# YukunXia/SuperPoint-Stereo-Visual-Odometry

Measured on AMD Instinct MI355X. Metric: stereo frames/sec (1241x376 KITTI), higher is better.
Workload: dtype f32

## Files before the change

### superpoint-stereo-visual-odometry_amd/csrc/conv_wino4.hip.h

```cpp
#pragma once
#include <hip/hip_runtime.h>
#include <stdint.h>
#include <type_traits>
#include <utility>
#include <vector>
#include "conv_mfma.hip.h"

#ifndef WINO4_LEAD
#define WINO4_LEAD 6
#endif
#ifndef WINO4_PRIO
#define WINO4_PRIO 1
#endif
#ifndef WINO4_H1_STEPS
#define WINO4_H1_STEPS 6
#endif
#ifndef WINO4_H1_START
#define WINO4_H1_START 3
#endif
#ifndef WINO4_H1_STRIDE
#define WINO4_H1_STRIDE 5
#endif
#ifndef WINO4_H2_START
#define WINO4_H2_START 4
#endif
#ifndef WINO4_H2_STRIDE
#define WINO4_H2_STRIDE 8
#endif
#ifndef WINO4_ITEM_LEAD
#define WINO4_ITEM_LEAD 6
#endif
#ifndef WINO4_ABL
#define WINO4_ABL 0
#endif

#ifndef SPVO_STATIC_BANDS
#define SPVO_STATIC_BANDS 1
#endif

namespace spvo {

template <int TB>
struct Wino4TileT {
  static constexpr int CK = 4, TH = 8 * TB, TW = 32, LW = TW + 8, LH = TH + 2, NT = 16 * TB, NTH = 256 * TB;
  static constexpr int IN_FLOATS = CK * LH * LW;
  static constexpr int U_FLOATS = 36 * CK * CO_TILE;
  static constexpr int V_FLOATS = 10 * TB * 64 * 4;
  static constexpr int RAW_OFF = 0, U_OFF = 2 * IN_FLOATS, V_OFF = U_OFF + 2 * U_FLOATS;
  static constexpr int LDS_BYTES = (V_OFF + 2 * V_FLOATS) * 4 + 16;
};
using Wino4Tile = Wino4TileT<2>;

inline std::vector<float> pack_conv_weights_wino4(const float *w, const float *bias, int cout, int cin) {
  constexpr int CK = Wino4Tile::CK;
  const int co_tiles = (cout + CO_TILE - 1) / CO_TILE, nch = cin / CK;
  std::vector<float> out((size_t)co_tiles * nch * Wino4Tile::U_FLOATS + (size_t)co_tiles * CO_TILE, 0.f);
  static const double G[6][3] = {{0.25, 0, 0}, {-1.0 / 6, -1.0 / 6, -1.0 / 6}, {-1.0 / 6, 1.0 / 6, -1.0 / 6},
                                 {1.0 / 24, 1.0 / 12, 1.0 / 6}, {1.0 / 24, -1.0 / 12, 1.0 / 6}, {0, 0, 1}};
  for (int ct = 0; ct < co_tiles; ++ct)
    for (int o = 0; o < CO_TILE; ++o) {
      const int co = ct * CO_TILE + o;
      if (co >= cout) continue;
      out[(size_t)co_tiles * nch * Wino4Tile::U_FLOATS + co] = bias[co];
// ... 1 lines not shown
        const float *g = w + ((size_t)co * cin + ci) * 9;
        double t[6][3];
        for (int a = 0; a < 6; ++a)
          for (int k = 0; k < 3; ++k) t[a][k] = G[a][0] * g[0 * 3 + k] + G[a][1] * g[1 * 3 + k] + G[a][2] * g[2 * 3 + k];
        float *slab = out.data() + ((size_t)ct * nch + ci / CK) * Wino4Tile::U_FLOATS;
        const int lane = 16 * (ci % CK) + (o & 15), cq = o >> 4;
        for (int a = 0; a < 6; ++a)
          for (int b = 0; b < 6; ++b) {
            const int pos = 18 * (b / 3) + 3 * a + b % 3;
            slab[(((pos >> 2) * 4 + cq) * 64 + lane) * 4 + (pos & 3)] = (float)(t[a][0] * G[b][0] + t[a][1] * G[b][1] + t[a][2] * G[b][2]);
          }
      }
    }
  return out;
}

__device__ __forceinline__ void wino4_in6(const float x0, const float x1, const float x2, const float x3, const float x4, const float x5, float (&o)[6]) {
  const float e = fmaf(-4.f, x2, x4), od = fmaf(-4.f, x1, x3), e2 = x4 - x2, o2 = x3 - x1;
  o[0] = fmaf(4.f, x0, fmaf(-5.f, x2, x4));
  o[1] = e + od;
  o[2] = e - od;
  o[3] = fmaf(2.f, o2, e2);
  o[4] = fmaf(-2.f, o2, e2);
  o[5] = fmaf(4.f, x1, fmaf(-5.f, x3, x5));
}
__device__ __forceinline__ void wino4_out4(const float m0, const float m1, const float m2, const float m3, const float m4, const float m5, float (&y)[4]) {
  const float a = m1 + m2, b = m1 - m2, c = m3 + m4, d = m3 - m4;
  y[0] = (m0 + a) + c;
  y[1] = fmaf(2.f, d, b);
  y[2] = fmaf(4.f, c, a);
  y[3] = fmaf(8.f, d, b) + m5;
}

typedef float wino4_f32x2 __attribute__((ext_vector_type(2)));
__device__ __forceinline__ void wino4_out4(const wino4_f32x2 m0, const wino4_f32x2 m1, const wino4_f32x2 m2, const wino4_f32x2 m3, const wino4_f32x2 m4,
                                           const wino4_f32x2 m5, wino4_f32x2 (&y)[4]) {
  const wino4_f32x2 a = m1 + m2, b = m1 - m2, c = m3 + m4, d = m3 - m4;
  y[0] = (m0 + a) + c;
  y[1] = __builtin_elementwise_fma(wino4_f32x2{2.f, 2.f}, d, b);
  y[2] = __builtin_elementwise_fma(wino4_f32x2{4.f, 4.f}, c, a);
  y[3] = __builtin_elementwise_fma(wino4_f32x2{8.f, 8.f}, d, b) + m5;
}

constexpr int wino4_b_piece(int p) { return 5 * (p / 18) + ((p % 18) >> 2); }
constexpr bool wino4_slot_reads_a(int q) { return (q & 3) == 0; }
constexpr bool wino4_slot_reads_b(int q) { return q == 0 || wino4_b_piece(q) != wino4_b_piece(q - 1); }
constexpr int wino4_reads_before(int q_end) {
  int n = 0;
  for (int q = 0; q < q_end && q < 36; ++q) n += (wino4_slot_reads_a(q) ? 1 : 0) + (wino4_slot_reads_b(q) ? 1 : 0);
  return n;
}
constexpr int wino4_first_slot_b(int piece) { return 18 * (piece / 5) + 4 * (piece % 5); }
constexpr int wino4_wait_count(int p, int lead) {
  const int issued = wino4_reads_before(p + lead);
  const int qa = p & ~3, qb = wino4_first_slot_b(wino4_b_piece(p));
  const int ia = wino4_reads_before(qa);
  const int ib = wino4_reads_before(qb) + (wino4_slot_reads_a(qb) ? 1 : 0);
  const int n = issued - 1 - (ia > ib ? ia : ib);
  return n < 0 ? 0 : (n > 15 ? 15 : n);
}
template <class F, int... P>
__device__ __forceinline__ void wino4_for_each(F &&f, std::integer_sequence<int, P...>) { (f(std::integral_constant<int, P>{}), ...); }

template <bool POOL, bool RELU, int TAG = 0, int TB = 2, int ITEM = 2>
__global__ __launch_bounds__(256 * TB, TB) void conv_wino4_kernel(const ConvArgs a) {
  using T = Wino4TileT<TB>;
  constexpr int CK = T::CK, LW = T::LW, LH = T::LH, LW4 = LW / 4, NTH = T::NTH;
  constexpr int IN_V4 = T::IN_FLOATS / 4;
  constexpr int U_V4 = T::U_FLOATS / 4;
  constexpr bool NEW_ITEM = ITEM != 0 && !(WINO4_ABL & 8);
  constexpr int NIT_U = (U_V4 + NTH - 1) / NTH;
  typedef float f32x2 __attribute__((ext_vector_type(2)));
  typedef float f32x4v __attribute__((ext_vector_type(4)));

  extern __shared__ __attribute__((aligned(16))) float smem[];

  const int tid = threadIdx.x;
  const int lane = tid & 63;
  const int c16 = lane & 15, g4 = lane >> 4;
  const int wave = __builtin_amdgcn_readfirstlane(tid >> 6);
  const int cq = wave & 3, tb = wave >> 2;
  const size_t in_plane = (size_t)a.in_hp * a.in_wp;
  const size_t out_plane = (size_t)a.out_hp * a.out_wp;
  const int n_tiles = a.tiles_x * a.tiles_y * a.co_tiles * a.batch;

  struct TileRef { const float *in_base, *w_base; int x0, y0, ct, img; };
  auto decode = [&](int id) {
    TileRef t;
    const int tx = id % a.tiles_x;
    id /= a.tiles_x;
    const int ty = id % a.tiles_y;
    id /= a.tiles_y;
    t.ct = id % a.co_tiles;
    t.img = id / a.co_tiles;
    t.x0 = tx * T::TW;
    t.y0 = ty * T::TH;
    t.in_base = a.in + ((size_t)t.img * a.in_ctot + a.in_coff) * in_plane + (size_t)(t.y0 + PADY - 1) * a.in_wp + (t.x0 + PADX - 4);
    t.w_base = a.wpack + (size_t)t.ct * a.n_chunks * T::U_FLOATS;
    return t;
  };

  auto raw_piece_off = [&](int idx) {
    idx = min(idx, IN_V4 - 1);
    const int ci = idx / (LH * LW4);
    const int rem = idx - ci * (LH * LW4);
    const int r = rem / LW4;
    const int q = rem - r * LW4;
    return 4u * (unsigned)(ci * (int)in_plane + r * a.in_wp + q * 4);
  };
  constexpr int R0 = NTH - 256;
  unsigned roff0 = raw_piece_off(tid), roff1 = raw_piece_off(NTH + (tid - R0));
  const bool raw2 = tid >= R0 && NTH + (tid - R0) < IN_V4;
  auto issue_raw = [&](const TileRef &t, int chunk, float *buf) {
    const char *inb = reinterpret_cast<const char *>(t.in_base + (size_t)chunk * CK * in_plane);
    glds16(reinterpret_cast<const float *>(inb + roff0), buf + (wave * 64) * 4);
    if (raw2) glds16(reinterpret_cast<const float *>(inb + roff1), buf + (NTH + (wave - R0 / 64) * 64) * 4);
  };
  unsigned uoff = 16u * (unsigned)tid;
  auto issue_u = [&](const TileRef &t, int chunk, float *buf) {
    const char *wb = reinterpret_cast<const char *>(t.w_base + (size_t)chunk * T::U_FLOATS);
#pragma unroll
    for (int it = 0; it < NIT_U; ++it)
      if (it < NIT_U - 1 || tid < U_V4 - (NIT_U - 1) * NTH) glds16(reinterpret_cast<const float *>(wb + (uoff + 16u * NTH * it)), buf + (it * NTH + wave * 64) * 4);
  };
  auto issue_raw2 = [&](const TileRef &t, int chunk, float *buf) {
    const char *inb = reinterpret_cast<const char *>(t.in_base + (size_t)chunk * CK * in_plane);
    glds16_sv(inb, roff0, buf + (wave * 64) * 4);
    if (raw2) glds16_sv(inb, roff1, buf + (NTH + (wave - R0 / 64) * 64) * 4);
  };
  auto issue_u2 = [&](const TileRef &t, int chunk, float *buf) {
    const char *wb = reinterpret_cast<const char *>(t.w_base + (size_t)chunk * T::U_FLOATS);
#pragma unroll
    for (int it = 0; it < NIT_U; ++it)
      if (it < NIT_U - 1 || tid < U_V4 - (NIT_U - 1) * NTH) glds16_sv(wb + (size_t)16 * NTH * it, uoff, buf + (it * NTH + wave * 64) * 4);
  };

  const int x_ci = TB == 2 ? (wave & 3) : 2 * (wave & 1) + ((lane >> 4) & 1), x_tile = TB == 2 ? (lane & 31) : (lane & 15), x_h = lane >> 5;
  const int x_trow = x_tile >> 3, x_tcol = x_tile & 7;
  const int raw_off = x_ci * (LH * LW) + (4 * x_trow + 3 * x_h) * LW + 4 * x_tcol + 3;
  const int v_off = x_h * (1280 * TB) + (x_tile >> 4) * 256 + (16 * x_ci + (x_tile & 15)) * 4;
  float xr[3][6];
  f32x4v xa[3];
  float xs0[3], xs1[3];
  f32x2 xs2[3];
  auto xf_step = [&](const float *raw, float *vb, int st) {
    if (st < 3) {
      const float *d = raw + raw_off + st * LW;
      xs0[st] = d[0];
      xa[st] = *reinterpret_cast<const f32x4v *>(d + 1);
      xs1[st] = d[5];
    } else if (st < 6) {
      const int r = st - 3;
      wino4_in6(xs0[r], xa[r][0], xa[r][1], xa[r][2], xa[r][3], xs1[r], xr[r]);
    } else if (st == 6) {
#pragma unroll
      for (int r = 0; r < 3; ++r)
#pragma unroll
        for (int c = 0; c < 3; ++c) {
          typedef unsigned u32x2s __attribute__((ext_vector_type(2)));
          const u32x2s sw = __builtin_amdgcn_permlane32_swap(__float_as_uint(xr[r][c]), __float_as_uint(xr[r][c + 3]), false, false);
          xr[r][c] = __uint_as_float(sw[0]);
          xr[r][c + 3] = __uint_as_float(sw[1]);
        }
    } else {
      const int c = st - 7;
      float o[6];
      wino4_in6(xr[0][c], xr[1][c], xr[2][c], xr[0][c + 3], xr[1][c + 3], xr[2][c + 3], o);
// ... 21 lines not shown
  };
  auto all_done = [&]() {
    if (a.sched && tid == 0 && atomicAdd(a.sched + 8, 1) == (int)gridDim.x - 1)
      for (int k = 0; k < 9; ++k) a.sched[k] = 0;
  };
  int *const sched_slot = reinterpret_cast<int *>(smem + (T::LDS_BYTES - 16) / 4);
  int tile_id = SPVO_STATIC_BANDS ? wgs_before(band) + ((int)blockIdx.x >> 3) : (int)blockIdx.x;
  if (a.sched) {
    tile_id = band_lo(band) + (blockIdx.x >> 3);
    if (tile_id >= band_hi(band)) {
      if (tid == 0) *sched_slot = steal();
      __syncthreads();
      tile_id = *sched_slot;
      __syncthreads();
    }
  }
  if (tile_id >= n_tiles) {
    all_done();
    return;
  }
  TileRef cur = decode(tile_id);

  int nxt_id = tile_id + gridDim.x;
  int dyn_fetch = 0;
  struct Cursor { TileRef t; int chunk, id; };
  auto advance = [&](Cursor &q) {
    if (++q.chunk == a.n_chunks) {
      asm volatile("" ::: "memory");
      q.chunk = 0;
      q.id = a.sched ? nxt_id : q.id + (int)gridDim.x;
      if (q.id < n_tiles) q.t = decode(q.id);
    }
  };
  Cursor cu{cur, 0, tile_id};
  issue_raw(cu.t, 0, smem + T::RAW_OFF);
  issue_u(cu.t, 0, smem + T::U_OFF);
  advance(cu);
  if (cu.id < n_tiles) issue_raw(cu.t, cu.chunk, smem + T::RAW_OFF + T::IN_FLOATS);
  Cursor cr = cu;
  advance(cr);
  asm volatile("s_waitcnt vmcnt(0)\n\ts_barrier" ::: "memory");
  if (wave < 2 * TB) {
#pragma unroll
    for (int st = 0; st < 10; ++st) xf_step(smem + T::RAW_OFF, smem + T::V_OFF, st);
  } else {
#pragma unroll
    for (int st = 0; st < WINO4_H1_STEPS; ++st) xf_step(smem + T::RAW_OFF + T::IN_FLOATS, smem + T::V_OFF + T::V_FLOATS, st);
  }
  asm volatile("s_waitcnt lgkmcnt(0)\n\ts_barrier" ::: "memory");
  if (cr.id < n_tiles) issue_raw(cr.t, cr.chunk, smem + T::RAW_OFF);
  advance(cr);

#ifdef WINO_STAMPS
  unsigned long long st_dma = 0, st_bar = 0, st_mfma = 0, st_epi = 0, st_items = 0, st_post = 0, st_bar_xf = 0, st_mfma_xf = 0;
  const unsigned long long st_t0 = __builtin_amdgcn_s_memtime(), st_r0 = __builtin_amdgcn_s_memrealtime();
  int st_c = 0;
#endif
  int k = 0;
  bool drained = false;
  constexpr unsigned OOB = 0xFFFFFFFFu;

  while (tile_id < n_tiles) {
    if (a.sched) {
      if (tid == 0) dyn_fetch = band_lo(band) + band_wgs(band) + atomicAdd(a.sched + band, 1);
    } else {
      nxt_id = tile_id + gridDim.x;
    }

    f32x4v acc[36];
    auto item = [&](auto first_tag, bool publish) {
      constexpr bool FIRST = decltype(first_tag)::value;
      const bool XF = NEW_ITEM ? (((wave >> TB) ^ k) & 1) == 0 : __builtin_amdgcn_readfirstlane((wave >> TB) == (k & 1) ? 1 : 0) != 0;
#ifdef WINO_STAMPS
      const unsigned long long ts0 = __builtin_amdgcn_s_memtime();
#endif
      if (!drained) asm volatile("s_waitcnt vmcnt(0)" ::: "memory");
      drained = false;
#ifdef WINO_STAMPS
      const unsigned long long ts1 = __builtin_amdgcn_s_memtime();
#endif
      if (publish && tid == 0) *sched_slot = dyn_fetch < band_hi(band) ? dyn_fetch : n_tiles;
      asm volatile("s_waitcnt lgkmcnt(0)\n\ts_barrier" ::: "memory");
      if (publish) nxt_id = __builtin_amdgcn_readfirstlane(*sched_slot);
#ifdef WINO_STAMPS
      const unsigned long long ts2 = __builtin_amdgcn_s_memtime();
      st_dma += ts1 - ts0; st_bar += ts2 - ts1;
      if (st_c == 1) st_post += ts1 - ts0;
      if (XF) st_bar_xf += ts2 - ts1;
#endif
      const float *ub = smem + T::U_OFF + (k & 1) * T::U_FLOATS;
      const float *vb = smem + T::V_OFF + (k & 1) * T::V_FLOATS;
      float *u_next = smem + T::U_OFF + ((k + 1) & 1) * T::U_FLOATS;
      const float *raw_next2 = smem + T::RAW_OFF + (k & 1) * T::IN_FLOATS;
      float *raw_next3 = smem + T::RAW_OFF + ((k + 1) & 1) * T::IN_FLOATS;
      float *v_next = smem + T::V_OFF + ((k + 1) & 1) * T::V_FLOATS;
      const f32x4v *ub4 = reinterpret_cast<const f32x4v *>(ub) + a_lane;
      const f32x4v *vb4 = reinterpret_cast<const f32x4v *>(vb) + b_lane;
      if constexpr (NEW_ITEM) {
        constexpr int LEAD = WINO4_ITEM_LEAD;
        static_assert(LEAD >= 1 && LEAD <= 36, "WINO4_ITEM_LEAD");
        static_assert(WINO4_PRIO <= 1, "the other priority schedules exist in the ITEM = 0 form only");
        f32x4v av[9], bv[10];
        f32x2 bh[2];
        static_assert(WINO4_H1_STEPS >= 6, "the row reads and the row pass that waits for them run in one item");
        const int xf_s = ((wave >> TB) ^ k ^ 1) & 1;
        auto is_xf = [xf_s]() __attribute__((always_inline)) { int t = xf_s; asm volatile("" : "+s"(t)); return t != 0; };
        const unsigned ra = (unsigned)(uintptr_t)(const __attribute__((address_space(3))) void *)(raw_next2 + raw_off);
        const unsigned ua = (unsigned)(uintptr_t)(const __attribute__((address_space(3))) void *)ub4;
        const unsigned va = (unsigned)(uintptr_t)(const __attribute__((address_space(3))) void *)vb4;
        auto read_slot = [&av, &bv, &bh, ua, va](auto qc) __attribute__((always_inline)) {
          constexpr int q = decltype(qc)::value;
          if constexpr (q < 36 && wino4_slot_reads_a(q)) asm volatile("ds_read_b128 %0, %1 offset:%2" : "=v"(av[q >> 2]) : "v"(ua), "n"((q >> 2) * 256 * 16));
          constexpr int j = wino4_b_piece(q < 36 ? q : 35);
          if constexpr (q < 36 && wino4_slot_reads_b(q) && j % 5 == 4) asm volatile("ds_read_b64 %0, %1 offset:%2" : "=v"(bh[j / 5]) : "v"(va), "n"(j * 64 * TB * 16));
          if constexpr (q < 36 && wino4_slot_reads_b(q) && j % 5 != 4) asm volatile("ds_read_b128 %0, %1 offset:%2" : "=v"(bv[j]) : "v"(va), "n"(j * 64 * TB * 16));
        };
        auto step = [&](auto pc) __attribute__((always_inline)) {
          constexpr int p = decltype(pc)::value;
          constexpr int ph = p / 18, pq = p % 18, pos = 6 * (pq / 3) + 3 * ph + pq % 3, bj = wino4_b_piece(p);
          constexpr bool half = bj % 5 == 4;
          if constexpr (wino4_slot_reads_a(p) || wino4_slot_reads_b(p)) {
            if constexpr (half) asm volatile("s_waitcnt lgkmcnt(%2)" : "+v"(av[p >> 2]), "+v"(bh[bj / 5]) : "n"(wino4_wait_count(p, LEAD)));
            else asm volatile("s_waitcnt lgkmcnt(%2)" : "+v"(av[p >> 2]), "+v"(bv[bj]) : "n"(wino4_wait_count(p, LEAD)));
          }
          const float a_op = av[p >> 2][p & 3];
          float b_op;
          if constexpr (half) b_op = bh[bj / 5][pq & 3];
          else b_op = bv[bj][pq & 3];
#if WINO4_PRIO
          if constexpr (p == 0) asm volatile("s_setprio 3");
          if constexpr (p == 9) asm volatile("s_setprio 2");
          if constexpr (p == 18) asm volatile("s_setprio 1");
          if constexpr (p == 27) asm volatile("s_setprio 0");
#endif
          if (FIRST) acc[pos] = __builtin_amdgcn_mfma_f32_16x16x4f32(a_op, b_op, f32x4v{0.f, 0.f, 0.f, 0.f}, 0, 0, 0);
          else acc[pos] = __builtin_amdgcn_mfma_f32_16x16x4f32(a_op, b_op, acc[pos], 0, 0, 0);
          __builtin_amdgcn_sched_barrier(0);
          if (!(WINO4_ABL & 2) && p == 1 && cu.id < n_tiles) { if constexpr (ITEM == 2) issue_u2(cu.t, cu.chunk, u_next); else issue_u(cu.t, cu.chunk, u_next); }
          if (!(WINO4_ABL & 4) && p == 4 && cr.id < n_tiles) { if constexpr (ITEM == 2) issue_raw2(cr.t, cr.chunk, raw_next3); else issue_raw(cr.t, cr.chunk, raw_next3); }
          read_slot(std::integral_constant<int, p + LEAD>{});
          if constexpr (!(WINO4_ABL & 1) && p >= WINO4_H1_START && p < WINO4_H1_START + WINO4_H1_STEPS * WINO4_H1_STRIDE && (p - WINO4_H1_START) % WINO4_H1_STRIDE == 0) {
            constexpr int st = (p - WINO4_H1_START) / WINO4_H1_STRIDE;
            if (is_xf()) {
              if constexpr (st < 3) {
                asm volatile("ds_read2_b32 %0, %1 offset0:%2 offset1:%3" : "=v"(xs2[st]) : "v"(ra), "n"(st * LW), "n"(st * LW + 5));
                asm volatile("ds_read_b128 %0, %1 offset:%2" : "=v"(xa[st]) : "v"(ra), "n"((st * LW + 1) * 4));
              } else {
                if constexpr (st < 6) {
                  constexpr int p_rd = p - 3 * WINO4_H1_STRIDE;
                  constexpr int n = wino4_reads_before(p + LEAD + 1) - wino4_reads_before(p_rd + LEAD + 1) + 2 * (5 - st);
                  asm volatile("s_waitcnt lgkmcnt(%2)" : "+v"(xs2[st - 3]), "+v"(xa[st - 3]) : "n"(n > 15 ? 15 : n));
                  xs0[st - 3] = xs2[st - 3][0];
                  xs1[st - 3] = xs2[st - 3][1];
                }
                xf_step(raw_next2, v_next, st);
              }
            }
          }
          if constexpr (!(WINO4_ABL & 1) && p >= WINO4_H2_START && p < WINO4_H2_START + (10 - WINO4_H1_STEPS) * WINO4_H2_STRIDE && (p - WINO4_H2_START) % WINO4_H2_STRIDE == 0)
            if (!is_xf()) xf_step(raw_next2, v_next, WINO4_H1_STEPS + (p - WINO4_H2_START) / WINO4_H2_STRIDE);
          __builtin_amdgcn_sched_barrier(0);
        };
        wino4_for_each(read_slot, std::make_integer_sequence<int, LEAD>{});
        wino4_for_each(step, std::make_integer_sequence<int, 36>{});
      } else {
        constexpr int LEAD = WINO4_LEAD;
        f32x4v av[9], bv[10];
        auto b_piece = [](int p) { return 5 * (p / 18) + ((p % 18) >> 2); };
#pragma unroll
        for (int p = 0; p < ((WINO4_ABL & 8) ? 36 : LEAD); ++p) {
          if ((WINO4_ABL & 8) && k > 0) break;
          if ((p & 3) == 0) av[p >> 2] = ub4[(p >> 2) * 256];
          if (p == 0 || b_piece(p) != b_piece(p - 1)) bv[b_piece(p)] = vb4[b_piece(p) * (64 * TB)];
        }
#pragma unroll
        for (int p = 0; p < 36; ++p) {
          const int ph = p / 18, pq = p % 18, pos = 6 * (pq / 3) + 3 * ph + pq % 3;
          const float a_op = av[p >> 2][p & 3], b_op = bv[b_piece(p)][pq & 3];
#if WINO4_PRIO
#if WINO4_PRIO == 1
          if (p == 0) asm volatile("s_setprio 3");
          if (p == 9) asm volatile("s_setprio 2");
          if (p == 18) asm volatile("s_setprio 1");
          if (p == 27) asm volatile("s_setprio 0");
#elif WINO4_PRIO == 2
          if (p == 0) asm volatile("s_setprio 3");
          if (tb == 0) { if (p == 6) asm volatile("s_setprio 2"); if (p == 15) asm volatile("s_setprio 1"); if (p == 24) asm volatile("s_setprio 0"); }
          else { if (p == 12) asm volatile("s_setprio 2"); if (p == 24) asm volatile("s_setprio 1"); }
#elif WINO4_PRIO == 3
          if (p == 0) asm volatile("s_setprio 1");
          if (p == 18) asm volatile("s_setprio 0");
#elif WINO4_PRIO == 4
          if (tb == 0) { if (p == 0) asm volatile("s_setprio 2"); if (p == 12) asm volatile("s_setprio 1"); if (p == 24) asm volatile("s_setprio 0"); }
          else { if (p == 0) asm volatile("s_setprio 3"); if (p == 12) asm volatile("s_setprio 2"); if (p == 24) asm volatile("s_setprio 1"); }
#endif
#endif
          if (FIRST) acc[pos] = __builtin_amdgcn_mfma_f32_16x16x4f32(a_op, b_op, f32x4v{0.f, 0.f, 0.f, 0.f}, 0, 0, 0);
          else acc[pos] = __builtin_amdgcn_mfma_f32_16x16x4f32(a_op, b_op, acc[pos], 0, 0, 0);
          __builtin_amdgcn_sched_barrier(0);
          if (!(WINO4_ABL & 2) && p == 1 && cu.id < n_tiles) issue_u(cu.t, cu.chunk, u_next);
          if (!(WINO4_ABL & 4) && p == 4 && cr.id < n_tiles) issue_raw(cr.t, cr.chunk, raw_next3);
          const int q = p + LEAD;
          if (!(WINO4_ABL & 8) && q < 36) {
            if ((q & 3) == 0) av[q >> 2] = ub4[(q >> 2) * 256];
            if (b_piece(q) != b_piece(q - 1)) bv[b_piece(q)] = vb4[b_piece(q) * (64 * TB)];
          }
          if (!(WINO4_ABL & 1) && XF && p >= WINO4_H1_START && p < WINO4_H1_START + WINO4_H1_STEPS * WINO4_H1_STRIDE && (p - WINO4_H1_START) % WINO4_H1_STRIDE == 0)
            xf_step(raw_next2, v_next, (p - WINO4_H1_START) / WINO4_H1_STRIDE);
          if (!(WINO4_ABL & 1) && !XF && p >= WINO4_H2_START && p < WINO4_H2_START + (10 - WINO4_H1_STEPS) * WINO4_H2_STRIDE && (p - WINO4_H2_START) % WINO4_H2_STRIDE == 0)
            xf_step(raw_next2, v_next, WINO4_H1_STEPS + (p - WINO4_H2_START) / WINO4_H2_STRIDE);
          __builtin_amdgcn_sched_barrier(0);
        }
      }
      advance(cu);
      advance(cr);
      ++k;
#ifdef WINO_STAMPS
      { const unsigned long long dt = __builtin_amdgcn_s_memtime() - ts2; st_mfma += dt; if (XF) st_mfma_xf += dt; }
      ++st_items; ++st_c;
#endif
    };
#ifdef WINO_STAMPS
    st_c = 0;
#endif
    item(std::true_type{}, false);
    for (int c = 1; c < a.n_chunks; ++c) item(std::false_type{}, a.sched != nullptr && c == 1);

#ifdef WINO_STAMPS
    const unsigned long long te0 = __builtin_amdgcn_s_memtime();
#endif
    asm volatile("s_waitcnt vmcnt(0)" ::: "memory");
    drained = true;

    const int co0 = cur.ct * CO_TILE + cq * 16 + 4 * g4;
    float *co_base = a.out + (((size_t)cur.img * a.out_ctot + a.out_coff) + (size_t)cur.ct * CO_TILE + cq * 16) * out_plane;
    const __amdgpu_buffer_rsrc_t rsrc = __builtin_amdgcn_make_buffer_rsrc(co_base, 0, 0x7FFFFFFF, 0x00020000);
    const int oplane = (int)out_plane;
    const int kmax = a.cout - co0;
    const float *bias_p = a.wpack + (size_t)a.co_tiles * a.n_chunks * T::U_FLOATS + min(co0, a.cout - 1);
    const int trow = 2 * tb + (c16 >> 3), tcol = c16 & 7;
    auto relu = [](float v) { return RELU ? __builtin_amdgcn_fmed3f(v, 0.f, __builtin_inff()) : v; };
    const int oy = cur.y0 + 4 * trow, ox = cur.x0 + 4 * tcol;
#pragma unroll
    for (int rp = 0; rp < 2; ++rp) {
      typedef wino4_f32x2 f32x2;
      const f32x2 bias_v = {bias_p[2 * rp < kmax ? 2 * rp : 0], bias_p[2 * rp + 1 < kmax ? 2 * rp + 1 : 0]};
      auto pr = [&](int p) { return f32x2{acc[p][2 * rp], acc[p][2 * rp + 1]}; };
      f32x2 z[6][4];
// ... 67 lines not shown
```

### superpoint-stereo-visual-odometry_amd/csrc/spvo_internal.hip.h

```cpp
#pragma once
#include <hip/hip_runtime.h>

#include <algorithm>
#include <cmath>
#include <cstdarg>
#include <cstdio>
#include <cstdlib>
#include <cstring>
#include <string>
#include <vector>
#include <deque>
#include <functional>
#include <time.h>

#include "../../include/spvo.h"
#include "spvo_types.hip.h"
#include "engine_file.h"

#pragma GCC visibility push(hidden)
#include "dev_buf.h"
namespace spvo { struct BriskLongPair; struct BriskShortPair; }
using namespace spvo;

#include "launch_segments.hip.h"
// ... 13 lines not shown
};
template <class T> using DevBuf = Buf<T, DevMem>;
template <class T> using PinBuf = Buf<T, PinnedMem>;

constexpr int RING = 8;
constexpr int MAX_INFLIGHT = 6;
constexpr int N_SLOTS = 16;
constexpr int N_BIN_SLOTS = 10;
constexpr int N_SIFT_SLOTS = 10;
constexpr int SIFT_SLOT_MAX = 32768;
constexpr int BIN_COUNTER_INTS = 16;
constexpr int HAM_KEY_SHIFT = 22;

struct Tensor {
  int ch = 0, level = 0, H = 0, W = 0, hp = 0, wp = 0;
  bool nhwc = false;
  bool f16 = false;
  bool i8 = false;
  bool s3 = false;
  float scale = 0.f;
  float *d = nullptr;
  float *dr[RING] = {};
  size_t per_image = 0;
};

struct Op {
  int type = 0, in = 0, out = 0, out_c_off = 0, in_c_off = 0, cin = 0, cout = 0, ks = 0, flags = 0;
  int ck = 0, n_chunks = 0, co_tiles = 0, wr = 0, wc = 0;
  int residual = 0;
  bool merged = false;
  bool wino = false;
  bool wino_narrow = false;
  bool wino4 = false;
  int wino4_item = 2;
  bool dominant = false;
  float *d_w = nullptr, *d_b = nullptr, *d_bn_scale = nullptr, *d_bn_shift = nullptr;
  int *d_sched = nullptr;
  _Float16 *d_w16 = nullptr;
  int8_t *d_w8 = nullptr;
  unsigned short *d_ws3 = nullptr;
  int *d_wq32 = nullptr;
  int *d_wsel = nullptr;
  int fused_dw = -1;
  bool fused_stem = false;
  bool fused_away = false;
  float *d_qm = nullptr;
  float inv_s_out = 0.f, s_res = 0.f;
  double flops_per_image = 0;
  int stage = -1;
  mutable int launch_tiles = 0, launch_wgs = 0;
  mutable int launch_block = 0;
};

struct Stage {
  std::string name;
  double total_ms = 0;
  long long calls = 0;
  double flops = 0, bytes = 0;
  double flops_sum = 0, bytes_sum = 0;
};

struct Pending { int stage; hipEvent_t e0, e1; double flops = 0, bytes = 0; };

struct SlotState {
  int n = 0;
  bool filled = false;
  DevBuf<int> d_n;
// ... 642 lines not shown
```

### superpoint-stereo-visual-odometry_amd/csrc/spvo_net_f32.hip

```cpp
#include "spvo_internal.hip.h"
#include "conv_mfma.hip.h"
#include "conv_wino2.hip.h"
#include "conv_wino4.hip.h"
#include "heads.hip.h"

namespace spvo_int {

int prepare_conv_f32(spvo_ctx *c, unsigned i, const float *w, const float *b) {
  Op &op = c->ops[i];
  const Tensor &ti = c->tensors[op.in];
  const bool bn = op.flags & FLAG_BN, add = op.flags & FLAG_ADD, pool = op.flags & FLAG_POOL;
  if (op.cin == 1) {
    if (pool || add) return fail(c, SPVO_ERR_IO, "op %u: single-channel-input layers have no pooling / residual form", i);
    return upload_stem(c, op, w, b);
  }
  op.ck = choose_variant(c, op, ti);
  {
    const bool wino_on = tuning("winograd", 1) != 0;
    const long wtiles = (long)((ti.W + WinoTile::TW - 1) / WinoTile::TW) * ((ti.H + WinoTile::TH - 1) / WinoTile::TH) * op.co_tiles * c->cfg.max_batch;
    const long min_tiles = tuning("winograd_min_tiles", 3 * c->num_cus / 4);
    const bool eligible = wino_on && op.ks == 3 && !bn && !add && (op.cin % WinoTile::CK) == 0 && (!pool || ((ti.H % 2) == 0 && (ti.W % 2) == 0));
    op.wino = eligible && wtiles >= min_tiles;
    if (eligible && !op.wino && tuning("wino_narrow", 1) && (op.cout % 32) == 0 && 3 * wtiles >= min_tiles) op.wino = op.wino_narrow = true;
  }
  const bool dynamic_tiles = tuning("wino_dynamic", 1) != 0;
  int rc;
  if (op.wino && !op.wino_narrow && (op.cin % Wino4Tile::CK) == 0 && (((ti.H | ti.W) & 1) == 0 || !pool) && tuning("wino4", 1)) {
    const long t4 = (long)((ti.W + Wino4Tile::TW - 1) / Wino4Tile::TW) * ((ti.H + Wino4Tile::TH - 1) / Wino4Tile::TH) * op.co_tiles * c->cfg.max_batch;
    if (t4 >= tuning("wino4_min_tiles", 3 * c->num_cus / 4)) {
      op.wino4 = true;
      op.wino4_item = (int)tuning("wino4_item", 2);
      op.ck = Wino4Tile::CK;
      op.n_chunks = op.cin / Wino4Tile::CK;
      if ((rc = upload(c, &op.d_w, pack_conv_weights_wino4(w, b, op.cout, op.cin)))) return rc;
      return dynamic_tiles ? dev_alloc(c, &op.d_sched, 16) : SPVO_OK;
    }
  }
  if (op.wino) {
    op.ck = WinoTile::CK;
    op.n_chunks = op.cin / op.ck;
    if (op.wino_narrow) op.co_tiles = op.cout / 32;
    if ((rc = upload(c, &op.d_w, pack_conv_weights_wino2(w, b, op.cout, op.cin, op.wino_narrow ? 32 : CO_TILE)))) return rc;
    return dynamic_tiles ? dev_alloc(c, &op.d_sched, 16) : SPVO_OK;
  }
  if (op.cin % op.ck) return fail(c, SPVO_ERR_IO, "op %u: cin %d is not a multiple of %d", i, op.cin, op.ck);
  op.n_chunks = op.cin / op.ck;
  std::vector<float> bp((size_t)op.co_tiles * CO_TILE, 0.f);
  for (int o = 0; o < op.cout; ++o) bp[o] = b[o];
  if ((rc = upload(c, &op.d_w, pack_conv_weights(w, b, op.cout, op.cin, op.ks, op.ck)))) return rc;
  return upload(c, &op.d_b, bp);
}

int fuse_tail_f32(spvo_ctx *c, const float *payload, const EngineOp &rp, const EngineOp &rd) {
  const Op &pb = c->ops[c->head_start], &db = c->ops[c->head_start + 1];
  const bool plain = tail_is_plain(c, HEADS_CIN) && !c->tensors[pb.in].nhwc && !c->tensors[db.in].nhwc && !pb.merged && !db.merged &&
                     c->tensors[pb.in].f16 == c->fp16 && c->tensors[db.in].f16 == c->fp16 && (!c->fp16 || ((pb.in_c_off | db.in_c_off) % 8) == 0);
  if (!plain) return SPVO_OK;
  const int rc = upload(c, &c->d_heads_w, pack_heads_weights(payload + rp.w_off, payload + rp.b_off, pb.cout, payload + rd.w_off, payload + rd.b_off, c->fp16));
  if (!rc) c->heads_fused = true;
  return rc;
}

template <int KS, int CK, int WR, int WC, bool POOL, bool RELU, int EPI = 0, int MINW = 1, int TAG = 0>
int launch_conv_instance(spvo_ctx *c, const ConvArgs &args, hipStream_t stream) {
// ... 49 lines not shown

template <bool POOL, bool RELU, int TAG, int ITEM>
int launch_conv_wino4_instance(spvo_ctx *c, const ConvArgs &args, hipStream_t stream) {
  static bool ready[64] = {};
  const int dev = c->cfg.device & 63;
  auto k = conv_wino4_kernel<POOL, RELU, TAG, 2, ITEM>;
  if (!ready[dev]) {
    HIP_TRY(c, hipFuncSetAttribute((const void *)k, hipFuncAttributeMaxDynamicSharedMemorySize, Wino4Tile::LDS_BYTES));
    ready[dev] = true;
  }
  const int n_tiles = args.tiles_x * args.tiles_y * args.co_tiles * args.batch;
  const int rounds = (n_tiles + c->num_cus - 1) / c->num_cus;
  const int grid = (n_tiles + rounds - 1) / rounds;
  ConvArgs a2 = args;
  if (rounds < 2 || args.n_chunks < 5) a2.sched = nullptr;
  hipLaunchKernelGGL(k, dim3(grid), dim3(512), Wino4Tile::LDS_BYTES, stream, a2);
  HIP_TRY(c, hipGetLastError());
  return SPVO_OK;
}

template <int ITEM>
int launch_conv_wino4_sel(spvo_ctx *c, const ConvArgs &args, bool relu, bool pool, bool dominant, hipStream_t stream) {
  if (dominant && relu) return pool ? launch_conv_wino4_instance<true, true, 1, ITEM>(c, args, stream) : launch_conv_wino4_instance<false, true, 1, ITEM>(c, args, stream);
  if (pool) return relu ? launch_conv_wino4_instance<true, true, 0, ITEM>(c, args, stream) : launch_conv_wino4_instance<true, false, 0, ITEM>(c, args, stream);
  return relu ? launch_conv_wino4_instance<false, true, 0, ITEM>(c, args, stream) : launch_conv_wino4_instance<false, false, 0, ITEM>(c, args, stream);
}

int launch_conv_wino4(spvo_ctx *c, const ConvArgs &a, int batch, bool relu, bool pool, bool dominant, int item, hipStream_t stream) {
  ConvArgs args = a;
  args.tiles_x = (a.W + Wino4Tile::TW - 1) / Wino4Tile::TW;
  args.tiles_y = (a.H + Wino4Tile::TH - 1) / Wino4Tile::TH;
  args.batch = batch;
  if (pool && ((a.H | a.W) & 1)) return fail(c, SPVO_ERR_INVALID, "F(4x4) kernel: pooled layer with odd size");
  if (item >= 2) return launch_conv_wino4_sel<2>(c, args, relu, pool, dominant, stream);
  return item == 1 ? launch_conv_wino4_sel<1>(c, args, relu, pool, dominant, stream) : launch_conv_wino4_sel<0>(c, args, relu, pool, dominant, stream);
}

int launch_conv_wino(spvo_ctx *c, const ConvArgs &a, int batch, bool relu, bool pool, bool dominant, bool narrow, hipStream_t stream) {
  ConvArgs args = a;
  args.tiles_x = (a.W + WinoTile::TW - 1) / WinoTile::TW;
  args.tiles_y = (a.H + WinoTile::TH - 1) / WinoTile::TH;
  args.batch = batch;
  return launch_conv_wino_sel(c, args, relu, pool, dominant, narrow, stream);
}

int launch_conv(spvo_ctx *c, const Op &op, int img0, int batch, hipStream_t stream) {
  const Tensor &ti = c->tensors[op.in];
  const Tensor &to = c->tensors[op.out];
  const float *tin = ring_ptr(c, ti, img0);
  float *tout = ring_ptr(c, to, img0);
  const bool relu = op.flags & FLAG_RELU, pool = op.flags & FLAG_POOL;
  const int epi = (op.flags & FLAG_BN) ? 1 : (op.flags & FLAG_ADD) ? 2 : 0;
  if (op.type == OP_DWCONV) {
    dim3 grid((ti.W + 255) / 256, (ti.H + 3) / 4, batch * op.cout);
    if (relu)
      hipLaunchKernelGGL(dwconv3x3_kernel<true>, grid, dim3(256), 0, stream, tin, tout, op.d_w, op.d_b, op.cout, ti.H, ti.W, ti.hp, ti.wp);
    else
      hipLaunchKernelGGL(dwconv3x3_kernel<false>, grid, dim3(256), 0, stream, tin, tout, op.d_w, op.d_b, op.cout, ti.H, ti.W, ti.hp, ti.wp);
    HIP_TRY(c, hipGetLastError());
    return SPVO_OK;
  }
  if (op.cin == 1) {
    dim3 grid((ti.W + 63) / 64, (ti.H + 3) / 4, batch);
#define SPVO_FIRST(KS, RELU) hipLaunchKernelGGL((conv_first_kernel<KS, RELU>), grid, dim3(256), 0, stream, tin, tout, op.d_w, op.d_b, \
                                                op.d_bn_scale, op.d_bn_shift, ti.H, ti.W, ti.hp, ti.wp, to.ch, op.out_c_off, op.cout, 0)
    if (op.ks == 3 && !op.d_bn_scale) {
      dim3 g4((ti.W + 255) / 256, (ti.H + 3) / 4, batch);
// ... 149 lines not shown
```

Before: 1592.

## Add item-3 Winograd F(4x4) path with persistent pointers and LDS address rotation

Adds a new kernel variant (ITEM=3, now the default) that keeps running global pointers for the filter and input DMA instead of recomputing them from tile descriptors, toggles the transform role and LDS buffer addresses by arithmetic swaps, and moves the priority setting and a sched barrier next to the lgkm waits. It also writes the row input transform as hand-scheduled inline assembly and stores transformed values directly to LDS. The aim is to cut scalar/vector address arithmetic and register pressure in the MFMA main loop. This adds opaque asm constraints that could hinder compiler scheduling and brings correctness risk in the pointer-advance logic.

```diff
diff --git a/superpoint-stereo-visual-odometry_amd/csrc/conv_wino4.hip.h b/superpoint-stereo-visual-odometry_amd/csrc/conv_wino4.hip.h
--- a/superpoint-stereo-visual-odometry_amd/csrc/conv_wino4.hip.h
+++ b/superpoint-stereo-visual-odometry_amd/csrc/conv_wino4.hip.h
@@ -29,6 +29,9 @@
 #endif
 #ifndef WINO4_ITEM_LEAD
 #define WINO4_ITEM_LEAD 6
+#endif
+#ifndef WINO4_ITEM3_STEPS
+#define WINO4_ITEM3_STEPS 31
 #endif
 #ifndef WINO4_ABL
 #define WINO4_ABL 0
@@ -96,6 +99,30 @@
   y[3] = fmaf(8.f, d, b) + m5;
 }
 
+__device__ __forceinline__ void wino4_in6_written_out(const float x0, const float x1, const float x2, const float x3, const float x4, const float x5, float (&o)[6]) {
+  float t, u;
+  asm("v_fma_f32 %6, -4.0, %10, %12\n\t"
+      "v_fma_f32 %7, -4.0, %9, %11\n\t"
+      "v_fmamk_f32 %0, %10, 0xc0a00000, %12\n\t"
+      "v_fmamk_f32 %5, %11, 0xc0a00000, %13\n\t"
+      "v_add_f32 %1, %6, %7\n\t"
+      "v_sub_f32 %2, %6, %7\n\t"
+      "v_sub_f32 %6, %12, %10\n\t"
+      "v_sub_f32 %7, %11, %9\n\t"
+      "v_fma_f32 %0, 4.0, %8, %0\n\t"
+      "v_fma_f32 %5, 4.0, %9, %5\n\t"
+      "v_fma_f32 %3, 2.0, %7, %6\n\t"
+      "v_fma_f32 %4, -2.0, %7, %6"
+      : "=&v"(o[0]), "=&v"(o[1]), "=&v"(o[2]), "=&v"(o[3]), "=&v"(o[4]), "=&v"(o[5]), "=&v"(t), "=&v"(u)
+      : "v"(x0), "v"(x1), "v"(x2), "v"(x3), "v"(x4), "v"(x5));
+}
+
+__device__ __forceinline__ void wino4_opaque_base(const char *&uniform_base) { asm volatile("" : "+s"(uniform_base)); }
+__device__ __forceinline__ void wino4_glds16_run(const char *opaque_uniform_base, unsigned &lane_off, float *lds_wave_base) {
+  asm volatile("" : "+v"(lane_off));
+  glds16(reinterpret_cast<const float *>(opaque_uniform_base + lane_off), lds_wave_base);
+}
+
 typedef float wino4_f32x2 __attribute__((ext_vector_type(2)));
 __device__ __forceinline__ void wino4_out4(const wino4_f32x2 m0, const wino4_f32x2 m1, const wino4_f32x2 m2, const wino4_f32x2 m3, const wino4_f32x2 m4,
                                            const wino4_f32x2 m5, wino4_f32x2 (&y)[4]) {
@@ -126,13 +153,16 @@
 template <class F, int... P>
 __device__ __forceinline__ void wino4_for_each(F &&f, std::integer_sequence<int, P...>) { (f(std::integral_constant<int, P>{}), ...); }
 
-template <bool POOL, bool RELU, int TAG = 0, int TB = 2, int ITEM = 2>
+template <bool POOL, bool RELU, int TAG = 0, int TB = 2, int ITEM = 3>
 __global__ __launch_bounds__(256 * TB, TB) void conv_wino4_kernel(const ConvArgs a) {
   using T = Wino4TileT<TB>;
   constexpr int CK = T::CK, LW = T::LW, LH = T::LH, LW4 = LW / 4, NTH = T::NTH;
   constexpr int IN_V4 = T::IN_FLOATS / 4;
   constexpr int U_V4 = T::U_FLOATS / 4;
   constexpr bool NEW_ITEM = ITEM != 0 && !(WINO4_ABL & 8);
+  constexpr int STEPS = !NEW_ITEM ? 0 : ITEM == 3 ? (WINO4_ITEM3_STEPS) : ITEM >= 16 ? ITEM - 16 : 0;
+  constexpr bool S_PTR = (STEPS & 1) != 0, S_ROLE = (STEPS & 2) != 0, S_WAIT = (STEPS & 4) != 0, S_LDS = (STEPS & 8) != 0, S_ROW = (STEPS & 16) != 0;
+  constexpr bool DMA_SV = ITEM >= 2;
   constexpr int NIT_U = (U_V4 + NTH - 1) / NTH;
   typedef float f32x2 __attribute__((ext_vector_type(2)));
   typedef float f32x4v __attribute__((ext_vector_type(4)));
@@ -197,6 +227,23 @@
 #pragma unroll
     for (int it = 0; it < NIT_U; ++it)
       if (it < NIT_U - 1 || tid < U_V4 - (NIT_U - 1) * NTH) glds16_sv(wb + (size_t)16 * NTH * it, uoff, buf + (it * NTH + wave * 64) * 4);
+  };
+  const char *wp3 = nullptr, *rp3 = nullptr;
+  constexpr int U_TAIL3 = T::U_FLOATS * 4 - (NIT_U - 1) * 16 * NTH, U_LAST_WAVES3 = (U_V4 - (NIT_U - 1) * NTH) / 64;
+  static_assert((U_V4 - (NIT_U - 1) * NTH) % 64 == 0, "the last filter piece by whole waves");
+  auto lds_ptr3 = [](unsigned lds) { return (float *)(__attribute__((address_space(3))) float *)(uintptr_t)lds; };
+  auto issue_raw3 = [&](unsigned lds) {
+    wino4_opaque_base(rp3);
+    wino4_glds16_run(rp3, roff0, lds_ptr3(lds));
+    if (raw2) wino4_glds16_run(rp3, roff1, lds_ptr3(lds + (NTH - R0) * 16));
+  };
+  auto issue_u3 = [&](unsigned lds) {
+#pragma unroll
+    for (int it = 0; it < NIT_U; ++it) {
+      if (it) wp3 += 16 * NTH;
+      wino4_opaque_base(wp3);
+      if (it < NIT_U - 1 || wave < U_LAST_WAVES3) wino4_glds16_run(wp3, uoff, lds_ptr3(lds + it * NTH * 16));
+    }
   };
 
   const int x_ci = TB == 2 ? (wave & 3) : 2 * (wave & 1) + ((lane >> 4) & 1), x_tile = TB == 2 ? (lane & 31) : (lane & 15), x_h = lane >> 5;
@@ -284,6 +331,18 @@
       if (q.id < n_tiles) q.t = decode(q.id);
     }
   };
+  auto advance3 = [&](Cursor &q, const char *&p, long step, bool filters) {
+    p += step;
+    if (++q.chunk == a.n_chunks) {
+      asm volatile("" ::: "memory");
+      q.chunk = 0;
+      q.id = a.sched ? nxt_id : q.id + (int)gridDim.x;
+      if (q.id < n_tiles) {
+        q.t = decode(q.id);
+        p = filters ? reinterpret_cast<const char *>(q.t.w_base) : reinterpret_cast<const char *>(q.t.in_base);
+      }
+    }
+  };
   Cursor cu{cur, 0, tile_id};
   issue_raw(cu.t, 0, smem + T::RAW_OFF);
   issue_u(cu.t, 0, smem + T::U_OFF);
@@ -311,6 +370,31 @@
   int k = 0;
   bool drained = false;
   constexpr unsigned OOB = 0xFFFFFFFFu;
+
+  auto lds_addr = [](const void *p) { return (unsigned)(uintptr_t)(const __attribute__((address_space(3))) void *)p; };
+  const int grp3 = (wave >> TB) & 1;
+  int xf3 = grp3 ^ 1;
+  unsigned lds_u3 = lds_addr(smem + T::U_OFF + T::U_FLOATS + wave * 256);
+  unsigned lds_raw3 = lds_addr(smem + T::RAW_OFF + T::IN_FLOATS + wave * 256);
+  const unsigned lds_u_swap3 = 2 * lds_u3 - T::U_FLOATS * 4, lds_raw_swap3 = 2 * lds_raw3 - T::IN_FLOATS * 4;
+  unsigned ua3 = lds_addr(reinterpret_cast<const f32x4v *>(smem + T::U_OFF) + a_lane);
+  unsigned va3 = lds_addr(reinterpret_cast<const f32x4v *>(smem + T::V_OFF) + b_lane);
+  unsigned ua_swap3 = 2 * ua3 + T::U_FLOATS * 4, va_swap3 = 2 * va3 + T::V_FLOATS * 4;
+  unsigned ra3 = lds_addr(smem + T::RAW_OFF + grp3 * T::IN_FLOATS + raw_off);
+  unsigned vst3 = lds_addr(smem + T::V_OFF + grp3 * T::V_FLOATS + v_off);
+  if constexpr (S_LDS) asm volatile("" : "+v"(ua3), "+v"(va3), "+v"(ra3), "+v"(vst3), "+v"(ua_swap3), "+v"(va_swap3));
+  auto xf_store3 = [&](int c) {
+    float o[6];
+    wino4_in6(xr[0][c], xr[1][c], xr[2][c], xr[0][c + 3], xr[1][c + 3], xr[2][c + 3], o);
+    float __attribute__((address_space(3))) *vp = (float __attribute__((address_space(3))) *)(uintptr_t)vst3;
+#pragma unroll
+    for (int i = 0; i < 6; ++i) vp[((3 * i + c) >> 2) * (256 * TB) + ((3 * i + c) & 3)] = o[i];
+  };
+  if constexpr (S_PTR) {
+    wp3 = reinterpret_cast<const char *>(cu.t.w_base + (size_t)cu.chunk * T::U_FLOATS);
+    rp3 = reinterpret_cast<const char *>(cr.t.in_base + (size_t)cr.chunk * CK * in_plane);
+  }
+  const long raw_step3 = (long)(CK * in_plane * 4);
 
   while (tile_id < n_tiles) {
     if (a.sched) {
@@ -356,10 +440,13 @@
         f32x2 bh[2];
         static_assert(WINO4_H1_STEPS >= 6, "the row reads and the row pass that waits for them run in one item");
         const int xf_s = ((wave >> TB) ^ k ^ 1) & 1;
-        auto is_xf = [xf_s]() __attribute__((always_inline)) { int t = xf_s; asm volatile("" : "+s"(t)); return t != 0; };
-        const unsigned ra = (unsigned)(uintptr_t)(const __attribute__((address_space(3))) void *)(raw_next2 + raw_off);
-        const unsigned ua = (unsigned)(uintptr_t)(const __attribute__((address_space(3))) void *)ub4;
-        const unsigned va = (unsigned)(uintptr_t)(const __attribute__((address_space(3))) void *)vb4;
+        auto is_xf = [xf_s, &xf3]() __attribute__((always_inline)) {
+          if constexpr (S_ROLE) { asm volatile("" : "+s"(xf3)); return xf3 != 0; }
+          else { int t = xf_s; asm volatile("" : "+s"(t)); return t != 0; }
+        };
+        const unsigned ra = S_LDS ? ra3 : (unsigned)(uintptr_t)(const __attribute__((address_space(3))) void *)(raw_next2 + raw_off);
+        const unsigned ua = S_LDS ? ua3 : (unsigned)(uintptr_t)(const __attribute__((address_space(3))) void *)ub4;
+        const unsigned va = S_LDS ? va3 : (unsigned)(uintptr_t)(const __attribute__((address_space(3))) void *)vb4;
         auto read_slot = [&av, &bv, &bh, ua, va](auto qc) __attribute__((always_inline)) {
           constexpr int q = decltype(qc)::value;
           if constexpr (q < 36 && wino4_slot_reads_a(q)) asm volatile("ds_read_b128 %0, %1 offset:%2" : "=v"(av[q >> 2]) : "v"(ua), "n"((q >> 2) * 256 * 16));
@@ -371,7 +458,21 @@
           constexpr int p = decltype(pc)::value;
           constexpr int ph = p / 18, pq = p % 18, pos = 6 * (pq / 3) + 3 * ph + pq % 3, bj = wino4_b_piece(p);
           constexpr bool half = bj % 5 == 4;
-          if constexpr (wino4_slot_reads_a(p) || wino4_slot_reads_b(p)) {
+          constexpr bool waits_here = wino4_slot_reads_a(p) || wino4_slot_reads_b(p);
+          auto set_prio = []() __attribute__((always_inline)) {
+#if WINO4_PRIO
+            if constexpr (p == 0) asm volatile("s_setprio 3");
+            if constexpr (p == 9) asm volatile("s_setprio 2");
+            if constexpr (p == 18) asm volatile("s_setprio 1");
+            if constexpr (p == 27) asm volatile("s_setprio 0");
+#endif
+          };
+          if constexpr (S_WAIT && waits_here) {
+            set_prio();
+            if constexpr (half) asm volatile("s_waitcnt lgkmcnt(%2)" : : "v"(av[p >> 2]), "v"(bh[bj / 5]), "n"(wino4_wait_count(p, LEAD)));
+            else asm volatile("s_waitcnt lgkmcnt(%2)" : : "v"(av[p >> 2]), "v"(bv[bj]), "n"(wino4_wait_count(p, LEAD)));
+            __builtin_amdgcn_sched_barrier(0);
+          } else if constexpr (waits_here) {
             if constexpr (half) asm volatile("s_waitcnt lgkmcnt(%2)" : "+v"(av[p >> 2]), "+v"(bh[bj / 5]) : "n"(wino4_wait_count(p, LEAD)));
             else asm volatile("s_waitcnt lgkmcnt(%2)" : "+v"(av[p >> 2]), "+v"(bv[bj]) : "n"(wino4_wait_count(p, LEAD)));
           }
@@ -379,38 +480,48 @@
           float b_op;
           if constexpr (half) b_op = bh[bj / 5][pq & 3];
           else b_op = bv[bj][pq & 3];
-#if WINO4_PRIO
-          if constexpr (p == 0) asm volatile("s_setprio 3");
-          if constexpr (p == 9) asm volatile("s_setprio 2");
-          if constexpr (p == 18) asm volatile("s_setprio 1");
-          if constexpr (p == 27) asm volatile("s_setprio 0");
-#endif
+          if constexpr (!(S_WAIT && waits_here)) set_prio();
           if (FIRST) acc[pos] = __builtin_amdgcn_mfma_f32_16x16x4f32(a_op, b_op, f32x4v{0.f, 0.f, 0.f, 0.f}, 0, 0, 0);
           else acc[pos] = __builtin_amdgcn_mfma_f32_16x16x4f32(a_op, b_op, acc[pos], 0, 0, 0);
           __builtin_amdgcn_sched_barrier(0);
-          if (!(WINO4_ABL & 2) && p == 1 && cu.id < n_tiles) { if constexpr (ITEM == 2) issue_u2(cu.t, cu.chunk, u_next); else issue_u(cu.t, cu.chunk, u_next); }
-          if (!(WINO4_ABL & 4) && p == 4 && cr.id < n_tiles) { if constexpr (ITEM == 2) issue_raw2(cr.t, cr.chunk, raw_next3); else issue_raw(cr.t, cr.chunk, raw_next3); }
+          if (!(WINO4_ABL & 2) && p == 1 && cu.id < n_tiles) {
+            if constexpr (S_PTR) issue_u3(lds_u3);
+            else if constexpr (DMA_SV) issue_u2(cu.t, cu.chunk, u_next);
+            else issue_u(cu.t, cu.chunk, u_next);
+          }
+          if (!(WINO4_ABL & 4) && p == 4 && cr.id < n_tiles) {
+            if constexpr (S_PTR) issue_raw3(lds_raw3);
+            else if constexpr (DMA_SV) issue_raw2(cr.t, cr.chunk, raw_next3);
+            else issue_raw(cr.t, cr.chunk, raw_next3);
+          }
           read_slot(std::integral_constant<int, p + LEAD>{});
-          if constexpr (!(WINO4_ABL & 1) && p >= WINO4_H1_START && p < WINO4_H1_START + WINO4_H1_STEPS * WINO4_H1_STRIDE && (p - WINO4_H1_START) % WINO4_H1_STRIDE == 0) {
-            constexpr int st = (p - WINO4_H1_START) / WINO4_H1_STRIDE;
-            if (is_xf()) {
-              if constexpr (st < 3) {
-                asm volatile("ds_read2_b32 %0, %1 offset0:%2 offset1:%3" : "=v"(xs2[st]) : "v"(ra), "n"(st * LW), "n"(st * LW + 5));
-                asm volatile("ds_read_b128 %0, %1 offset:%2" : "=v"(xa[st]) : "v"(ra), "n"((st * LW + 1) * 4));
-              } else {
-                if constexpr (st < 6) {
-                  constexpr int p_rd = p - 3 * WINO4_H1_STRIDE;
-                  constexpr int n = wino4_reads_before(p + LEAD + 1) - wino4_reads_before(p_rd + LEAD + 1) + 2 * (5 - st);
-                  asm volatile("s_waitcnt lgkmcnt(%2)" : "+v"(xs2[st - 3]), "+v"(xa[st - 3]) : "n"(n > 15 ? 15 : n));
-                  xs0[st - 3] = xs2[st - 3][0];
-                  xs1[st - 3] = xs2[st - 3][1];
-                }
-                xf_step(raw_next2, v_next, st);
+          constexpr bool h1_slot = !(WINO4_ABL & 1) && p >= WINO4_H1_START && p < WINO4_H1_START + WINO4_H1_STEPS * WINO4_H1_STRIDE && (p - WINO4_H1_START) % WINO4_H1_STRIDE == 0;
+          constexpr bool h2_slot = !(WINO4_ABL & 1) && p >= WINO4_H2_START && p < WINO4_H2_START + (10 - WINO4_H1_STEPS) * WINO4_H2_STRIDE && (p - WINO4_H2_START) % WINO4_H2_STRIDE == 0;
+          auto h1 = [&](auto stc) __attribute__((always_inline)) {
+            constexpr int st = decltype(stc)::value;
+            if constexpr (st < 3) {
+              asm volatile("ds_read2_b32 %0, %1 offset0:%2 offset1:%3" : "=v"(xs2[st]) : "v"(ra), "n"(st * LW), "n"(st * LW + 5));
+              asm volatile("ds_read_b128 %0, %1 offset:%2" : "=v"(xa[st]) : "v"(ra), "n"((st * LW + 1) * 4));
+            } else {
+              if constexpr (st < 6) {
+                constexpr int p_rd = p - 3 * WINO4_H1_STRIDE;
+                constexpr int n = wino4_reads_before(p + LEAD + 1) - wino4_reads_before(p_rd + LEAD + 1) + 2 * (5 - st);
+                asm volatile("s_waitcnt lgkmcnt(%2)" : "+v"(xs2[st - 3]), "+v"(xa[st - 3]) : "n"(n > 15 ? 15 : n));
+                xs0[st - 3] = xs2[st - 3][0];
+                xs1[st - 3] = xs2[st - 3][1];
               }
+              if constexpr (S_ROW && st < 6) wino4_in6_written_out(xs0[st - 3], xa[st - 3][0], xa[st - 3][1], xa[st - 3][2], xa[st - 3][3], xs1[st - 3], xr[st - 3]);
+              else xf_step(raw_next2, v_next, st);
             }
-          }
-          if constexpr (!(WINO4_ABL & 1) && p >= WINO4_H2_START && p < WINO4_H2_START + (10 - WINO4_H1_STEPS) * WINO4_H2_STRIDE && (p - WINO4_H2_START) % WINO4_H2_STRIDE == 0)
-            if (!is_xf()) xf_step(raw_next2, v_next, WINO4_H1_STEPS + (p - WINO4_H2_START) / WINO4_H2_STRIDE);
+          };
+          auto h2 = [&](auto stc) __attribute__((always_inline)) {
+            constexpr int st = decltype(stc)::value;
+            if constexpr (S_LDS && st >= 7) xf_store3(st - 7);
+            else xf_step(raw_next2, v_next, st);
+          };
+          constexpr int st1 = (p - WINO4_H1_START) / WINO4_H1_STRIDE, st2 = WINO4_H1_STEPS + (p - WINO4_H2_START) / WINO4_H2_STRIDE;
+          if constexpr (h1_slot) { if (is_xf()) h1(std::integral_constant<int, st1>{}); }
+          if constexpr (h2_slot) { if (!is_xf()) h2(std::integral_constant<int, st2>{}); }
           __builtin_amdgcn_sched_barrier(0);
         };
         wino4_for_each(read_slot, std::make_integer_sequence<int, LEAD>{});
@@ -464,8 +575,20 @@
           __builtin_amdgcn_sched_barrier(0);
         }
       }
-      advance(cu);
-      advance(cr);
+      if constexpr (S_PTR) {
+        advance3(cu, wp3, U_TAIL3, true);
+        advance3(cr, rp3, raw_step3, false);
+        lds_u3 = lds_u_swap3 - lds_u3;
+        lds_raw3 = lds_raw_swap3 - lds_raw3;
+      } else {
+        advance(cu);
+        advance(cr);
+      }
+      if constexpr (S_ROLE) xf3 ^= 1;
+      if constexpr (S_LDS) {
+        ua3 = ua_swap3 - ua3;
+        va3 = va_swap3 - va3;
+      }
       ++k;
 #ifdef WINO_STAMPS
       { const unsigned long long dt = __builtin_amdgcn_s_memtime() - ts2; st_mfma += dt; if (XF) st_mfma_xf += dt; }
diff --git a/superpoint-stereo-visual-odometry_amd/csrc/spvo_internal.hip.h b/superpoint-stereo-visual-odometry_amd/csrc/spvo_internal.hip.h
--- a/superpoint-stereo-visual-odometry_amd/csrc/spvo_internal.hip.h
+++ b/superpoint-stereo-visual-odometry_amd/csrc/spvo_internal.hip.h
@@ -69,7 +69,7 @@
   bool wino = false;
   bool wino_narrow = false;
   bool wino4 = false;
-  int wino4_item = 2;
+  int wino4_item = 3;
   bool dominant = false;
   float *d_w = nullptr, *d_b = nullptr, *d_bn_scale = nullptr, *d_bn_shift = nullptr;
   int *d_sched = nullptr;
diff --git a/superpoint-stereo-visual-odometry_amd/csrc/spvo_net_f32.hip b/superpoint-stereo-visual-odometry_amd/csrc/spvo_net_f32.hip
--- a/superpoint-stereo-visual-odometry_amd/csrc/spvo_net_f32.hip
+++ b/superpoint-stereo-visual-odometry_amd/csrc/spvo_net_f32.hip
@@ -29,7 +29,7 @@
     const long t4 = (long)((ti.W + Wino4Tile::TW - 1) / Wino4Tile::TW) * ((ti.H + Wino4Tile::TH - 1) / Wino4Tile::TH) * op.co_tiles * c->cfg.max_batch;
     if (t4 >= tuning("wino4_min_tiles", 3 * c->num_cus / 4)) {
       op.wino4 = true;
-      op.wino4_item = (int)tuning("wino4_item", 2);
+      op.wino4_item = (int)tuning("wino4_item", 3);
       op.ck = Wino4Tile::CK;
       op.n_chunks = op.cin / Wino4Tile::CK;
       if ((rc = upload(c, &op.d_w, pack_conv_weights_wino4(w, b, op.cout, op.cin)))) return rc;
@@ -145,7 +145,8 @@
   args.tiles_y = (a.H + Wino4Tile::TH - 1) / Wino4Tile::TH;
   args.batch = batch;
   if (pool && ((a.H | a.W) & 1)) return fail(c, SPVO_ERR_INVALID, "F(4x4) kernel: pooled layer with odd size");
-  if (item >= 2) return launch_conv_wino4_sel<2>(c, args, relu, pool, dominant, stream);
+  if (item >= 3) return launch_conv_wino4_sel<3>(c, args, relu, pool, dominant, stream);
+  if (item == 2) return launch_conv_wino4_sel<2>(c, args, relu, pool, dominant, stream);
   return item == 1 ? launch_conv_wino4_sel<1>(c, args, relu, pool, dominant, stream) : launch_conv_wino4_sel<0>(c, args, relu, pool, dominant, stream);
 }
 
```

Result: faster. 1633, median of 6 (+2.6%).
